# ArchDD/CPP-Raytracer-Rasterizer

Hardware: AMD Instinct MI355X
Metric: Mrays/s (primary+shadow) (higher is better)
Workload: dtype f32

## Files before the change

### cpp-raytracer-rasterizer_amd/capi/binned.cpp

```cpp
#include "capi.hpp"

namespace mirt {


int ensure_pairs(RtScratch &S, size_t cap)
{
    int r;
    if ((r = dev_realloc(&S.d_entries, cap)) || (r = dev_realloc(&S.d_pair_keys, cap)) || (r = dev_realloc(&S.d_pair_vals, cap)) ||
        (r = dev_realloc(&S.d_sorted_keys, cap)) || (r = dev_realloc(&S.d_tmp_vals, cap))) { S.cap_entries = 0; return r; }
    S.cap_entries = (uint32_t)cap;
    return MIRT_OK;
}

constexpr uint32_t BIN_MAX_KEYS = BUCKET_SORT_MAX_BUCKETS * 1024u - 1u;

void poll_pair_count(RtScratch &S)
{
    if (S.count_pending && hipEventQuery(S.ev_count) == hipSuccess) {
        S.known_pairs = *S.h_count; S.have_known = true; S.count_pending = false;
    }
    (void)hipGetLastError();
}

int bin_pass(RtScratch &S, BinSet bs, const OriginRow *cam_tab, const OriginRow *light_tab, uint32_t *counter, uint32_t *bin_off,
             bool fresh, uint32_t *npairs, bool may_guess = false)
{
    int rc;
    poll_pair_count(S);
    if (!fresh && may_guess && S.have_known && S.known_pairs > S.cap_used) fresh = true;
    const bool guess = fresh && may_guess && S.have_known;
    if (!S.d_entries || !S.cap_entries) {
        static const size_t initial = [] { const long v = env_int("MIRT_BIN_INITIAL_PAIRS", 0); return v > 0 ? (size_t)v : (size_t)1 << 20; }();
        if ((rc = ensure_pairs(S, initial))) return rc;
    }
    if (bs.nbins > BIN_MAX_KEYS) return fail(MIRT_ERR_INVALID_ARGUMENT, "binning: %u sort keys exceed the %u the bucket sort holds", bs.nbins, BIN_MAX_KEYS);
    bs.chunk_tris = 256;
    const dim3 bin_grid((unsigned)std::min<long long>((long long)((g.n + bs.chunk_tris - 1) / bs.chunk_tris) * bs.nframes, (long long)g.cu_count * 8));
    bs.counters = counter;
    const uint32_t nbuckets = bucket_sort_buckets(bs.nbins);
    if (nbuckets + 1 > S.cap_buckets) {
        S.cap_buckets = 0;
        if ((rc = dev_realloc(&S.d_bucket, (size_t)3 * (nbuckets + 1)))) return rc;
        HIP_TRY(hipMemsetAsync(S.d_bucket, 0, sizeof(uint32_t) * 3 * (nbuckets + 1), g.stream));
        S.cap_buckets = nbuckets + 1;
        S.bucket_dirty = false;
    }
    uint32_t *bcnt = S.d_bucket, *bbase = S.d_bucket + S.cap_buckets, *bcur = S.d_bucket + 2 * (size_t)S.cap_buckets;
    bs.bucket_cnt = bcnt; bs.nbuckets = nbuckets; bs.bucket_shift = bucket_sort_shift(bs.nbins);
    const size_t bin_lds = (size_t)nbuckets * sizeof(uint32_t);
    {
        static const bool once = [] {
            (void)hipFuncSetAttribute(reinterpret_cast<const void *>(&k_bin_pairs<512>), hipFuncAttributeMaxDynamicSharedMemorySize, 48 * 1024);
            (void)hipFuncSetAttribute(reinterpret_cast<const void *>(&k_bin_pairs<256>), hipFuncAttributeMaxDynamicSharedMemorySize, 48 * 1024);
            return true; }();
        (void)once;
    }
    static const int bin_wg_env = (int)env_int("MIRT_BIN_WG", 0);
    const int bin_wg = (bin_wg_env == 256 || bin_wg_env == 512) ? bin_wg_env : ((g.n < 400000 && g.in_flight >= 3) ? 256 : 512);
    if (guess) {
        const size_t want = (size_t)S.known_pairs + S.known_pairs / 2 + 4096;
        if (want > S.cap_entries) {
            HIP_TRY(hipStreamSynchronize(g.stream));
            if ((rc = ensure_pairs(S, want + want / 4))) return rc;
        }
    }
    bool publish_count = false;
    for (int attempt = 0; attempt < 2; attempt++) {
        static const uint32_t test_cap = [] { const long v = env_int("MIRT_TEST_PAIR_CAP", 0); return v > 0 ? (uint32_t)v : 0u; }();
        S.cap_used = (guess && test_cap && test_cap < S.cap_entries) ? test_cap : S.cap_entries;
        BinPairs pairs = { S.d_pair_keys, S.d_pair_vals, S.cap_used };
        bs.entries = S.d_entries; bs.cap_entries = S.cap_used;
        if (attempt) HIP_TRY(hipMemsetAsync(counter, 0, 4, g.stream));
        if (attempt || S.bucket_dirty) HIP_TRY(hipMemsetAsync(S.d_bucket, 0, sizeof(uint32_t) * 3 * (size_t)S.cap_buckets, g.stream));
        S.bucket_dirty = true;
        if (bin_wg == 256) hipLaunchKernelGGL(k_bin_pairs<256>, bin_grid, dim3(256), bin_lds, g.stream, g.d_tris, cam_tab, light_tab, g.n, bs, pairs);
        else hipLaunchKernelGGL(k_bin_pairs<512>, bin_grid, dim3(512), bin_lds, g.stream, g.d_tris, cam_tab, light_tab, g.n, bs, pairs);
        if (!fresh) break;
        if (guess) {
            if (!S.h_count) {
                HIP_TRY(hipHostMalloc(reinterpret_cast<void **>(&S.h_count), 64, hipHostMallocDefault));
                HIP_TRY(hipEventCreateWithFlags(&S.ev_count, hipEventDisableTiming));
            }
            if (!S.count_pending) publish_count = true;
            *npairs = S.known_pairs;
            break;
        }
        uint32_t total = 0;
        HIP_TRY(hipStreamSynchronize(g.stream));
        HIP_TRY(hipMemcpy(&total, counter, 4, hipMemcpyDeviceToHost));
        *npairs = total;
        S.known_pairs = total; S.have_known = true;
// ... 285 lines not shown
        bs.frame0.nshell = okr ? ns : 1;
        bs.frame0.shell_d0 = (float)dn;
        bs.frame0.shell_iw = okr ? (float)(ns / (df - dn)) : 0.0f;
    }
    const uint32_t cam_keys = (uint32_t)bs.frame0.nbu * (uint32_t)band_tile_rows * (uint32_t)bs.frame0.nshell;
    const int tshells = transient ? light_shells_for(nlights, cube_bins, 0u) : 1;
    const uint32_t per_light = 6u * (uint32_t)(cube_bins * cube_bins) * (uint32_t)tshells;
    bs.nbins = cam_keys;
    if (bs.nbins + 1 > S.cap_bins) {
        const size_t cap = (size_t)bs.nbins + 1;
        HIP_TRY(hipStreamSynchronize(g.stream));
        if ((rc = dev_realloc(&S.d_bin_off, cap))) { S.cap_bins = 0; return rc; }
        S.cap_bins = (uint32_t)cap;
        S.bin_key_valid = false;
    }
    if (!S.d_bin_counters) { HIP_TRY(hipMalloc(reinterpret_cast<void **>(&S.d_bin_counters), 512)); HIP_TRY(hipMemsetAsync(S.d_bin_counters, 0, 512, g.stream)); }
    if (S.sel_n != g.n) {
        HIP_TRY(hipStreamSynchronize(g.stream));
        S.sel_n = 0;
        if ((rc = dev_realloc(&S.d_sel, (size_t)g.n))) return rc;
        S.sel_n = g.n;
        S.bin_key_valid = false;
    }
    bs.bin_off = S.d_bin_off;

    uint64_t key = 0xcbf29ce484222325ull ^ g.scene_version;
    {
        auto mix = [&](const void *p, size_t nb) { const unsigned char *b = (const unsigned char *)p; for (size_t i = 0; i < nb; i++) { key ^= b[i]; key *= 0x100000001b3ull; } };
        mix(view, sizeof *view); mix(&y0, 4); mix(&y1, 4); mix(&g.n, 4); mix(&g.aa, 4);
    }
    const int bin_mode = 0;
// ... 18 lines not shown
        forked = !reuse && !side_off;
        if (forked) {
            HIP_TRY(hipEventRecord(ss.ev_fork, main_stream));
            HIP_TRY(hipStreamWaitEvent(ss.aux, ss.ev_fork, 0));
            g.stream = ss.aux;
        }
        rc = transient_light_pass(L, f, origins, nlights, cube_bins, tshells, per_light, lkey, &lights_kept, reuse ? g.d_hits : nullptr);
        g.stream = main_stream;
        if (rc) return rc;
        if (forked) HIP_TRY(hipEventRecord(ss.ev_join, ss.aux));
    }
    if (reuse) {
        if (!(transient && !lights_kept)) HIP_TRY(hipMemsetAsync(g.d_hits, 0, HIT_BYTES, g.stream));
        g.stats.bins_reused = 1;
    } else {
        S.sel_parity ^= 1;
        SelectOut so;
        memset(&so, 0, sizeof so);
        so.cam_tab = S.d_cam_tab; so.sel = S.d_sel;
        so.sel_count = S.d_bin_counters + SEL_COUNT0 + S.sel_parity; so.sel_count_next = S.d_bin_counters + SEL_COUNT0 + (S.sel_parity ^ 1);
        so.zero_hits = g.d_hits; so.zero_counter = S.d_bin_counters;
        if ((rc = hist_prepare(S, bs.frame0, &so))) return rc;
        const unsigned sel_grid = (unsigned)std::min<long long>(((long long)g.n + 1023) / 1024, (long long)g.cu_count);
        hipLaunchKernelGGL(k_prep_select, dim3(sel_grid), dim3(1024), 0, g.stream, g.d_tris, g.n, bs.frame0, so);
        if ((rc = hist_publish(S))) return rc;
        bs.sel = S.d_sel; bs.sel_count = so.sel_count;
        g.stats_sel_count = so.sel_count;
        if ((rc = bin_pass(S, bs, S.d_cam_tab, nullptr, S.d_bin_counters, S.d_bin_off, true, &S.bin_entries, may_guess))) return rc;
        S.last_bin_mode = bin_mode;
        S.bin_key = key;
        S.bin_key_valid = true;
        if ((size_t)order_seg > S.cap_order) {
            HIP_TRY(hipStreamSynchronize(g.stream));
            S.cap_order = 0;
            if ((rc = dev_realloc(&S.d_order, (size_t)ORDER_GROUPS * ORDER_CLASSES * order_seg))) return rc;
            S.cap_order = order_seg;
        }
        hipLaunchKernelGGL(k_tile_order, dim3((pairs_x + 63) / 64, (unsigned)(bs.frame0.j1 - bs.frame0.j0)), dim3(64), 0, g.stream, cam_off, bs.frame0.nshell,
                           bs.frame0.nbu, bs.frame0.j0, bs.frame0.j1, S.d_bin_counters, S.cap_used, S.d_order, order_seg);
    }
    if (forked) HIP_TRY(hipStreamWaitEvent(g.stream, ss.ev_join, 0));
    k_end(MIRT_K_BIN);

    bp->cam_off = cam_off;
    bp->tiles_x = bs.frame0.nbu;
    bp->cam_shells = bs.frame0.nshell;
    bp->order_seg = order_seg;
    bp->transient = transient;
    bp->cube_bins = cube_bins;
    bp->light_shells = transient ? tshells : g.lc.shells;
    return MIRT_OK;
}

int hist_only_pass(const mirt_view *view)
{
    int rc;
    g.stream = g.cur().stream;
    RtScratch &S = g.cur().rt;
    if (S.cam_tab_n != g.n) {
        S.cam_tab_n = 0;
        if ((rc = dev_realloc(&S.d_cam_tab, (size_t)g.n))) return rc;
        S.cam_tab_n = g.n;
    }
    if (S.sel_n != g.n) {
        HIP_TRY(hipStreamSynchronize(g.stream));
        S.sel_n = 0;
        if ((rc = dev_realloc(&S.d_sel, (size_t)g.n))) return rc;
        S.sel_n = g.n;
    }
    if (!S.d_bin_counters) { HIP_TRY(hipMalloc(reinterpret_cast<void **>(&S.d_bin_counters), 512)); HIP_TRY(hipMemsetAsync(S.d_bin_counters, 0, 512, g.stream)); }
    S.bin_key_valid = false;
    const BinFrameDesc fr = make_camera_frame(view, 0, 0, g.aa);
    SelectOut so;
    memset(&so, 0, sizeof so);
    so.cam_tab = S.d_cam_tab; so.sel = S.d_sel;
    so.sel_count = S.d_bin_counters + HIST_SEL_COUNT; so.sel_count_next = S.d_bin_counters + HIST_SEL_COUNT + 1;
    if ((rc = hist_prepare(S, fr, &so))) return rc;
    if (!g.hist_armed) return MIRT_OK;
    HIP_TRY(hipMemsetAsync(so.sel_count, 0, 4, g.stream));
    const unsigned sel_grid = (unsigned)std::min<long long>(((long long)g.n + 1023) / 1024, (long long)g.cu_count);
    if (sel_grid) hipLaunchKernelGGL(k_prep_select, dim3(sel_grid), dim3(1024), 0, g.stream, g.d_tris, g.n, fr, so);
    HIP_TRY(hipGetLastError());
    return hist_publish(S);
}

int binned_trace(const RtFrame &f, RtScratch &S, RtScratch &L, const BinnedPass &bp)
{
    const bool transient = bp.transient;
    RtTraceFrame tf;
    memset(&tf, 0, sizeof tf);
    tf.f = f;
    tf.f.cam_tab = S.d_cam_tab;
    tf.f.light_tab = transient ? L.d_light_tab : g.lc.d_light_tab;
    tf.f.unsafe = nullptr;
    tf.cam_off = bp.cam_off;
    tf.cam_entries = S.d_entries;
    tf.sel = S.d_sel; tf.sel_count = S.d_bin_counters + SEL_COUNT0 + S.sel_parity;
    static const int lazy_env = (int)env_int("MIRT_LAZY_GEO", -1);
    tf.lazy_geo = lazy_env >= 0 ? (lazy_env != 0) : (g.n >= 400000);
    tf.geo = g.d_geo;
    tf.shade = g.d_shade;
    tf.light_off = transient ? L.d_bin_off : g.lc.d_off;
    tf.light_rows = transient ? L.d_light_rows : g.lc.d_rows;
    tf.light_tri = transient ? L.d_entries : g.lc.d_row_tri;
    tf.light_frames = transient ? L.d_frames : g.lc.d_frames;
    tf.tiles_x = bp.tiles_x;
    tf.cube_bins = bp.cube_bins;
    tf.cam_shells = bp.cam_shells;
    tf.light_shells = bp.light_shells;
    tf.pair_count = S.d_bin_counters;
    tf.pair_cap = S.cap_used;
    tf.light_pair_count = transient ? L.d_bin_counters : nullptr;
    tf.light_pair_cap = L.cap_used;
    tf.order = S.d_order; tf.order_count = S.d_bin_counters + 16; tf.order_seg = bp.order_seg;
    const dim3 tgrid(ORDER_GROUPS * bp.order_seg);
    const size_t lds = rt_trace_lds_bytes(1);
    k_begin(MIRT_K_TRACE);
    g.pending_counted = g.profiling;
    if (f.aa > 1) {
        if (g.profiling) hipLaunchKernelGGL((k_rt_trace2<true, true>), tgrid, dim3(64), lds, g.stream, tf);
        else hipLaunchKernelGGL((k_rt_trace2<true, false>), tgrid, dim3(64), lds, g.stream, tf);
    } else {
        static const int waves5_env = (int)env_int("MIRT_TR_WAVES5", -1);
        const bool waves5 = waves5_env >= 0 ? (waves5_env != 0) : (g.n >= 400000 || g.in_flight <= 2);
        if (g.profiling) hipLaunchKernelGGL((k_rt_trace2<false, true>), tgrid, dim3(64), lds, g.stream, tf);
        else if (waves5) hipLaunchKernelGGL((k_rt_trace2<false, false, 5>), tgrid, dim3(64), lds, g.stream, tf);
        else hipLaunchKernelGGL((k_rt_trace2<false, false>), tgrid, dim3(64), lds, g.stream, tf);
    }
    k_end(MIRT_K_TRACE);
// ... 12 lines not shown
```

### cpp-raytracer-rasterizer_amd/capi/capi.hpp

```cpp
#pragma once

#include "../csrc/bin_sort.hpp"
#include "../csrc/comm.hpp"
#include "../csrc/cull.hpp"
#include "../csrc/dof.hpp"
#include "../csrc/rt_common.hpp"
#include "../csrc/raster_common.hpp"
#include "../csrc/rt_binned.hpp"
#include "../csrc/scan.hpp"
#include "env.hpp"

#include <cstdarg>
#include <cstdio>
#include <cstdlib>
#include <cstring>
#include <algorithm>
#include <cmath>
#include <vector>

#define MIRT_KERNEL __attribute__((global))

namespace mirt {

MIRT_KERNEL void k_prep_origin(const float *, int, const float *, v3, int, OriginRow *, OriginRow *, uint32_t *, unsigned long long *, uint32_t *);
template <int P> MIRT_KERNEL void k_rt_brute(const RtFrame);
template <int P> MIRT_KERNEL void k_rt_small(const RtFrame, int);
MIRT_KERNEL void k_rt_wave(const RtFrame);
struct RtTileFrame {
    RtFrame f;
    BinFrameDesc cam;
    int tiles_x, tiles_y;
    unsigned long long *clear_hits;
    float4 *tables;
};
MIRT_KERNEL void k_tile_tables(const RtTileFrame);
template <int TW, bool AA> MIRT_KERNEL void k_rt_tile2(const RtTileFrame);
template <int WG> MIRT_KERNEL void k_bin_pairs(const float *, const OriginRow *, const OriginRow *, int, BinSet, BinPairs);
struct TilePairRec { uint32_t tile, beg, nA, nB; };
constexpr int ORDER_CLASSES = 8, ORDER_GROUPS = 8;
struct RtTraceFrame {
    RtFrame f;
    const uint32_t *cam_off;
    const uint32_t *cam_entries;
    const GeoRow *geo;
    const ShadeRow *shade;
    const uint32_t *light_off;
    const LightRow *light_rows;
    const uint32_t *light_tri;
    const BinFrameDesc *light_frames;
    int tiles_x;
    int cube_bins;
    int cam_shells;
// ... 19 lines not shown
size_t rt_trace_lds_bytes(int waves);
int launch_raster(RasterFrame &f, RasterScratch &s, uint64_t scene_version, hipStream_t stream, hipEvent_t *ev, bool *ev_used);

extern char g_err[512];
int fail(int code, const char *fmt, ...);

#define HIP_TRY(expr)                                                                          \
    do {                                                                                       \
        hipError_t e_ = (expr);                                                                \
        if (e_ != hipSuccess)                                                                  \
            return fail(MIRT_ERR_HIP, "%s failed: %s (%s:%d)", #expr, hipGetErrorString(e_), __FILE__, __LINE__); \
    } while (0)

enum { EV_CALL0 = 0, EV_CALL1 = 1, EV_K0 = 2, EV_COUNT = 2 + 2 * 8 };
constexpr int MAX_FLIGHT = 4;
constexpr int SEL_COUNT0 = 80;
constexpr int HIST_SEL_COUNT = 82;
constexpr int HIST_RING = 4;
constexpr int HIST_SLOTS = HIST_RING + 1;
constexpr size_t HIT_BYTES = sizeof(unsigned long long) * HIT_SHARDS * HIT_SHARD_STRIDE;

struct RtScratch {
    OriginRow *d_cam_tab = nullptr;
    OriginRow *d_light_tab = nullptr;
    int cam_tab_n = 0, light_tab_n = 0, light_tab_lights = 0;
    float *d_origins = nullptr;
    uint32_t *d_flags = nullptr;
    BinFrameDesc *d_frames = nullptr;
    uint32_t *d_bin_off = nullptr, *d_bin_counters = nullptr;
    uint32_t *d_entries = nullptr;
    uint32_t *d_pair_keys = nullptr, *d_pair_vals = nullptr, *d_sorted_keys = nullptr;
    uint32_t *d_tmp_vals = nullptr;
// ... 6 lines not shown
    bool count_event_due = false;
    bool have_known = false;
    uint32_t known_pairs = 0;
    uint32_t cap_bins = 0, cap_entries = 0;
    uint32_t cap_used = 0;
    uint64_t bin_key = 0;
    uint32_t bin_entries = 0;
    bool bin_key_valid = false;
    LightRow *d_light_rows = nullptr;
    uint32_t cap_light_rows = 0;
    TilePairRec *d_order = nullptr;
    uint32_t cap_order = 0;
    int last_bin_mode = -1;
    uint32_t *d_sel = nullptr;
    int sel_n = 0;
    int sel_parity = 0;
    uint32_t *d_face_sel = nullptr;
    size_t cap_face_sel = 0;
    uint32_t *d_face_counts = nullptr;
    uint32_t *d_hist = nullptr;
    uint32_t *h_hist = nullptr;
    hipEvent_t ev_hist[HIST_SLOTS] = {};
    uint64_t hist_key[HIST_SLOTS] = {};
    uint64_t hist_seq[HIST_SLOTS] = {};
    int hist_rows[HIST_SLOTS] = {}, hist_shift[HIST_SLOTS] = {};
    int hist_next = 0;

    void forget_scene() { bin_key_valid = false; have_known = false; count_pending = false; }
    void release();
};

// ... 146 lines not shown
    int tiles_x, cam_shells;
    uint32_t order_seg;
    bool transient;
    int cube_bins, light_shells;
};
int binned_pass(const RtFrame &f, const mirt_view *view, RtScratch &S, RtScratch &L, const float *origins, int nlights, int y0, int y1, BinnedPass *bp);
int binned_trace(const RtFrame &f, RtScratch &S, RtScratch &L, const BinnedPass &bp);
bool rt_bins_whole_frame(const mirt_view *view, const mirt_light *lights, int nlights, int mode);
int hist_only_pass(const mirt_view *view);

int raster_enqueue(const mirt_view *view, const mirt_light *lights, int nlights, const float *indirect,
                   int y0, int y1, int row_origin, void *d_xrgb, int pitch_bytes, void *d_rgb, void *d_zinv,
                   void *d_index, void *d_fd = nullptr);
int cull_copy_wait_readers(int dst, hipStream_t st);

int hist_prepare(RtScratch &S, const BinFrameDesc &cam, SelectOut *so);
int hist_publish(RtScratch &S);
const uint32_t *hist_lookup(uint64_t max_key, int *rows, int *shift);
void current_bounds(int world, int W, int H, std::vector<int> &bounds);
unsigned part_tile_weight();
int plan_out(int world, int root, int width, int height, int nviews, int strip_rows, const int *bounds, uint64_t *root_offset,
             uint64_t *band_offset, uint64_t *bytes, int32_t *peer, int max_pieces);
int render_sharded(const mirt_view *views, int nviews, int root, void *d_frames, int pitch_bytes, bool raster,
                   const mirt_light *lights, int nlights, const float *indirect, int mode);

struct HostPlane { void *host; void **staging; size_t bpp; };
int ensure_staging(size_t px, const HostPlane *planes, int nplanes);
char *registered_alias(const void *host, size_t pitch, int H);
bool host_direct();
int copy_plane_interior(void *dst, int dst_pitch, const void *src, int src_pitch, int W, int H);
// ... 66 lines not shown
```

### cpp-raytracer-rasterizer_amd/capi/sharded.cpp

```cpp
#include "capi.hpp"

namespace mirt {

static bool hist_wanted() { return g.in_sharded ? g.hist_call : (g.want_hist || g.strip_rows == MIRT_PARTITION_WEIGHTED); }
static int hist_shift_for(int tile_rows) { int sh = 0; while (((tile_rows - 1) >> sh) + 1 > SEL_HIST_MAX) sh++; return sh; }
static int hist_slot(const RtScratch &S) { return g.in_sharded ? S.hist_next : HIST_RING; }
int hist_prepare(RtScratch &S, const BinFrameDesc &cam, SelectOut *so)
{
    g.hist_armed = false;
    if (!hist_wanted()) return MIRT_OK;
    if (!S.d_hist) {
        HIP_TRY(hipMalloc(reinterpret_cast<void **>(&S.d_hist), sizeof(uint32_t) * SEL_HIST_MAX));
        HIP_TRY(hipMemsetAsync(S.d_hist, 0, sizeof(uint32_t) * SEL_HIST_MAX, g.stream));
        HIP_TRY(hipHostMalloc(reinterpret_cast<void **>(&S.h_hist), sizeof(uint32_t) * SEL_HIST_MAX * HIST_SLOTS, hipHostMallocDefault));
        for (int i = 0; i < HIST_SLOTS; i++) HIP_TRY(hipEventCreateWithFlags(&S.ev_hist[i], hipEventDisableTiming));
    }
    so->hist = S.d_hist;
    so->hist_shift = hist_shift_for(cam.nbv);
    const int slot = hist_slot(S);
    S.hist_key[slot] = 0;
    S.hist_rows[slot] = ((cam.nbv - 1) >> so->hist_shift) + 1;
    S.hist_shift[slot] = so->hist_shift;
    g.hist_armed = true;
    return MIRT_OK;
// ... 160 lines not shown
```

### cpp-raytracer-rasterizer_amd/csrc/bin_bucket_sort.hip

```cpp
#include "bin_sort.hpp"

#include <algorithm>
#include <cstdlib>

namespace mirt {

constexpr int BS_PER_THREAD = 16;
constexpr int BS_CHUNK = 256 * BS_PER_THREAD;
constexpr int BS_LOCAL_PER_THREAD = 16;
constexpr int BS_MAX_SHIFT = 12;
constexpr int BS_MAX_BUCKET_KEYS = 1 << BS_MAX_SHIFT;

__device__ __forceinline__ uint32_t bs_block_scan(uint32_t v, uint32_t *s_wave , uint32_t *total)
{
    const int lane = threadIdx.x & 63, wave = threadIdx.x >> 6;
    uint32_t incl = v;
#pragma unroll
    for (int d = 1; d < 64; d <<= 1) {
        const uint32_t o = __shfl_up(incl, d);
        if (lane >= d) incl += o;
    }
    __syncthreads();
    if (lane == 63) s_wave[wave] = incl;
    __syncthreads();
// ... 64 lines not shown
__global__ __launch_bounds__(256) void k_bs_local(const uint32_t *__restrict__ keys, const uint32_t *__restrict__ vals,
                                                  const uint32_t *__restrict__ total_ptr, uint32_t cap,
                                                  const uint32_t *__restrict__ bucket_base, uint32_t nbins, int shift,
                                                  uint32_t *__restrict__ bucket_cnt, uint32_t *__restrict__ cursor,
                                                  uint32_t *__restrict__ bin_off, uint32_t *__restrict__ entries)
{
    __shared__ uint32_t s_cnt[BS_MAX_BUCKET_KEYS], s_wave[4];
    const uint32_t bucket = blockIdx.x;
    if (threadIdx.x == 0) { bucket_cnt[bucket] = 0u; cursor[bucket] = 0u; }
    if (*total_ptr > cap) return;
    const uint32_t beg = bucket_base[bucket], end = bucket_base[bucket + 1];
    const uint32_t nb = 1u << shift, mask = nb - 1u;
    for (uint32_t i = threadIdx.x; i < nb; i += 256) s_cnt[i] = 0u;
    __syncthreads();
    const bool small = end - beg <= 256u * BS_LOCAL_PER_THREAD;
    uint32_t lo[BS_LOCAL_PER_THREAD], v[BS_LOCAL_PER_THREAD], rank[BS_LOCAL_PER_THREAD];
    if (small) {
#pragma unroll
        for (int j = 0; j < BS_LOCAL_PER_THREAD; j++) {
            const uint32_t i = beg + threadIdx.x + 256u * j;
            lo[j] = 0xFFFFFFFFu; v[j] = 0u; rank[j] = 0u;
            if (i < end) { lo[j] = keys[i] & mask; v[j] = vals[i]; }
        }
#pragma unroll
        for (int j = 0; j < BS_LOCAL_PER_THREAD; j++)
            if (lo[j] != 0xFFFFFFFFu) rank[j] = atomicAdd(&s_cnt[lo[j]], 1u);
    } else {
        for (uint32_t i = beg + threadIdx.x; i < end; i += 256) atomicAdd(&s_cnt[keys[i] & mask], 1u);
    }
    __syncthreads();
    uint32_t carry = beg;
    for (uint32_t i0 = 0; i0 < nb; i0 += 256) {
        const uint32_t i = i0 + threadIdx.x;
        const uint32_t c = i < nb ? s_cnt[i] : 0u;
        uint32_t all;
        const uint32_t excl = carry + bs_block_scan(c, s_wave, &all);
        if (i < nb) {
            s_cnt[i] = excl;
            const uint32_t bin = (bucket << shift) + i;
            if (bin <= nbins) bin_off[bin] = excl;
        }
        carry += all;
    }
    __syncthreads();
    if (small) {
#pragma unroll
        for (int j = 0; j < BS_LOCAL_PER_THREAD; j++)
            if (lo[j] != 0xFFFFFFFFu) entries[s_cnt[lo[j]] + rank[j]] = v[j];
    } else {
        for (uint32_t i = beg + threadIdx.x; i < end; i += 256) {
            const uint32_t at = atomicAdd(&s_cnt[keys[i] & mask], 1u);
            entries[at] = vals[i];
        }
    }
}

int bucket_sort_shift(uint32_t nbins)
{
    int shift = 8;
    while (shift < BS_MAX_SHIFT && ((nbins + 1u + (1u << shift) - 1u) >> shift) > 1024u) shift++;
    while (shift > 4 && ((nbins + 1u + (1u << shift) - 1u) >> shift) < 512u) shift--;
    return shift;
}
// ... 21 lines not shown
```

### cpp-raytracer-rasterizer_amd/csrc/rt_binned.hip

```cpp
#include "rt_binned.hpp"

#include <float.h>

namespace mirt {

constexpr int BIN_L0 = BIN_COARSE * BIN_COARSE;

struct BinItem {
    float A0[4], A1[4], A2[4], Bu[4], Bv[4];
    float lou, hiu, lov, hiv;
};

__device__ __forceinline__ float bcastf(float v, int lane) { return __builtin_bit_cast(float, __builtin_amdgcn_readlane(__builtin_bit_cast(int, v), lane)); }

__device__ __forceinline__ float corner(float s, float lo, float hi) { return fmaxf(s * lo, s * hi); }

__device__ __forceinline__ bool cell_may_hit(const BinItem &u, const float (&A)[4], float I, float J, float K)
{
    bool ok = true;
#pragma unroll
    for (int k = 0; k < 4; k++) ok = ok && (__builtin_fmaf(J, u.Bv[k], __builtin_fmaf(I, u.Bu[k], A[k])) >= 0.0f);
    return ok && (I + K >= u.lou) && (I <= u.hiu) && (J + K >= u.lov) && (J <= u.hiv);
}

// ... 231 lines not shown
        for (int f = 0; f < 6; f++) {
            const unsigned long long m = __builtin_amdgcn_ballot_w64((keep >> f) & 1u);
            if (m) {
                uint32_t at0 = 0;
                if (lane == 0) at0 = atomicAdd(&s_fill[f], (uint32_t)__popcll(m));
                at0 = (uint32_t)__builtin_amdgcn_readfirstlane((int)at0);
                if ((keep >> f) & 1u) s_sel[f][at0 + (uint32_t)__popcll(m & ((1ull << lane) - 1ull))] = (uint32_t)i;
            }
        }
        __syncthreads();
    }
    flush();
}


template <int WG>
__global__ __launch_bounds__(WG) void k_bin_pairs(const float *__restrict__ tris15, const OriginRow *__restrict__ cam_tab,
                                                   const OriginRow *__restrict__ light_tab, int n, BinSet bs, BinPairs out)
{
    extern __shared__ uint32_t s_bucket[];
    __shared__ uint32_t s_keys[BIN_PAIR_BUF], s_vals[BIN_PAIR_BUF];
    __shared__ float4 s_A2[256], s_Bu[256], s_Bv[256], s_box[256];
    __shared__ uint32_t s_org[256];
    __shared__ uint32_t s_ni[256];
    __shared__ uint32_t s_tri[256];
    __shared__ uint32_t s_pre[257];
    __shared__ uint32_t s_wave[4];
    __shared__ uint32_t s_base, s_fill, s_valid;
    const int lane = threadIdx.x & 63, wave = threadIdx.x >> 6;
    const int chunk_tris = bs.chunk_tris;
    const int nchunks = (n + chunk_tris - 1) / chunk_tris;
    const bool listed = bs.sel != nullptr;
    const uint32_t nsel = listed ? min(*bs.sel_count, (uint32_t)n) : 0u;
    const int cam_chunk = (listed && nsel < 32768u) ? 64 : chunk_tris;
    const int ncam = listed ? (int)((nsel + (uint32_t)cam_chunk - 1u) / (uint32_t)cam_chunk) : 0;
    const int nrest = listed ? bs.nframes - 1 : bs.nframes;
    const bool faces_listed = bs.face_lists != nullptr;
    __shared__ uint32_t s_first[MAX_BIN_FRAMES + 1];
    if (faces_listed) {
        if (threadIdx.x == 0) {
            uint32_t run = 0;
            for (int ff = 0; ff < nrest; ff++) { s_first[ff] = run; run += (min(bs.face_counts[ff], (uint32_t)n) + (uint32_t)chunk_tris - 1u) / (uint32_t)chunk_tris; }
            s_first[nrest] = run;
        }
        __syncthreads();
    }
    const int nwork = ncam + (faces_listed ? (int)s_first[nrest] : nchunks * nrest);
    if (threadIdx.x == 0) { s_fill = 0u; s_valid = (uint32_t)BIN_PAIR_BUF; }
    if (bs.bucket_cnt)
        for (uint32_t b = threadIdx.x; b < bs.nbuckets; b += WG) s_bucket[b] = 0u;

    auto flush = [&]() {
// ... 50 lines not shown
        BinFrameGrid gr;
        gr.nbu = fr.nbu; gr.fj0 = fr.j0; gr.fj1 = fr.j1; gr.fbase = fr.base; gr.nshell = (uint32_t)max(fr.nshell, 1);
        gr.cells_x = (gr.nbu + BIN_L0 - 1) / BIN_L0; gr.cy0 = gr.fj0 / BIN_L0;
        gr.ncell = gr.cells_x * ((gr.fj1 + BIN_L0 - 1) / BIN_L0 - gr.cy0);
        const int nbu = gr.nbu, fj0 = gr.fj0, fj1 = gr.fj1;
        BinItem it;
        memset(&it, 0, sizeof it);
        int kind = 0;
#ifdef MIRT_BIN_STATS
        int dbg_state = 0;
#endif
        int i_lo = 0, i_hi = -1, j_lo = 0, j_hi = -1;
        unsigned long long cells = 0;
        uint32_t shell = 0;
        if (tri < (uint32_t)n && fj1 > fj0) {
            const OriginRow &row = (fr.tab == 0) ? cam_tab[tri] : light_tab[(size_t)(fr.tab - 1) * n + tri];
            shell = bin_shell_of(fr, row.r1.w);
            TriBinFns t = make_bin_fns(row, fr);
            add_bbox(t, tris15 + (size_t)15 * tri, fr);
#ifdef MIRT_BIN_STATS
            dbg_state = t.bstate == BOX_VALID ? 0 : (t.bstate == BOX_NONE ? 1 : 2);
#endif
            const float T = 1.6940658945086007e-21f;
            const bool both = fabsf(t.nb) < T || !(t.nb == t.nb);
            const float sgn = t.nb < 0.0f ? -1.0f : 1.0f;
            const EdgeFn *fn[4] = { &t.n, &t.p, &t.q, &t.s };
            const float inf = __builtin_huge_valf();
#pragma unroll
            for (int k = 0; k < 4; k++) {
                const float su = sgn * fn[k]->cu, sv = sgn * fn[k]->cv;
                const float base = sgn * fn[k]->c0 + fn[k]->m + su * fr.ulo + sv * fr.vlo;
// ... 24 lines not shown
                    const int cx = c % gr.cells_x, cy = gr.cy0 + c / gr.cells_x;
                    if (cell_may_hit(it, it.A0, (float)(cx * BIN_L0), (float)(cy * BIN_L0), (float)BIN_L0)) cells |= 1ull << c;
                }
                if (gr.ncell > 64) cells = ~0ull;
                if (!cells) kind = 0;
                if (kind == 2 && !both) {
                    BinLin G[4];
#pragma unroll
                    for (int k = 0; k < 4; k++) { G[k].a = sgn * fn[k]->c0 + fn[k]->m; G[k].bu = sgn * fn[k]->cu; G[k].bv = sgn * fn[k]->cv; }
                    const float u0 = fr.ulo + fr.pad_lo, u1 = fr.ulo + (float)nbu * fr.du + fr.pad_hi;
                    const float v0 = fr.vlo + (float)fj0 * fr.dv + fr.pad_lo, v1 = fr.vlo + (float)fj1 * fr.dv + fr.pad_hi;
                    if (bin_jointly_empty(G, u0, u1, v0, v1)) kind = 0;
                }
            }
        }



        STAMP(st_setup)
        const uint32_t ni = (uint32_t)(i_hi - i_lo + 1);
        const uint32_t nb = kind == 1 ? ni * (uint32_t)(j_hi - j_lo + 1) : 0u;
        uint32_t incl = nb;
#pragma unroll
        for (int d = 1; d < 64; d <<= 1) {
            const uint32_t o = __shfl_up(incl, d);
            if (lane >= d) incl += o;
        }
        __syncthreads();
        if (lane == 63 && wave < 4) s_wave[wave] = incl;
        if (kind == 1) {
            s_A2[threadIdx.x] = make_float4(it.A2[0], it.A2[1], it.A2[2], it.A2[3]);
            s_Bu[threadIdx.x] = make_float4(it.Bu[0], it.Bu[1], it.Bu[2], it.Bu[3]);
            s_Bv[threadIdx.x] = make_float4(it.Bv[0], it.Bv[1], it.Bv[2], it.Bv[3]);
            s_box[threadIdx.x] = make_float4(it.lou, it.hiu, it.lov, it.hiv);
            s_org[threadIdx.x] = (uint32_t)i_lo | ((uint32_t)j_lo << 16);
            s_ni[threadIdx.x] = ni | (shell << 8);
            s_tri[threadIdx.x] = tri;
        }
        __syncthreads();
        const uint32_t t0w = s_wave[0], t1w = s_wave[1], t2w = s_wave[2], t3w = s_wave[3];
        if (threadIdx.x < 256) s_pre[threadIdx.x] = (wave > 0 ? t0w : 0u) + (wave > 1 ? t1w : 0u) + (wave > 2 ? t2w : 0u) + incl - nb;
        const uint32_t T = t0w + t1w + t2w + t3w;
        if (threadIdx.x == 0) s_pre[256] = T;

#ifdef MIRT_BIN_STATS
        if (kind == 2) { atomicAdd(&bs.counters[11 + dbg_state], 1u); if (frame == 0) atomicAdd(&bs.counters[14], 1u); }
        if (threadIdx.x == 0) { atomicAdd(&bs.counters[8], T); atomicMax(&bs.counters[9], T); }
        { const unsigned long long md = __ballot(kind == 1); if (lane == 0) atomicAdd(&bs.counters[10], (uint32_t)__popcll(md)); }
#endif
        STAMP(st_prefix)
        constexpr int TPT = BIN_TESTS_PER_THREAD;
        for (uint32_t r0 = 0; r0 < T; r0 += WG * TPT) {
#ifdef MIRT_BIN_STAMPS
            st_nrounds++;
#endif
            __syncthreads();
            if (s_fill + (uint32_t)(WG * TPT) > (uint32_t)BIN_PAIR_BUF) flush();
            bool pass[TPT];
// ... 32 lines not shown
            if (cnt) {
                uint32_t at0 = 0;
                if (lane == 0) at0 = atomicAdd(&s_fill, cnt);
                at0 = (uint32_t)__builtin_amdgcn_readfirstlane((int)at0);
#pragma unroll
                for (int q = 0; q < TPT; q++)
                    if (pass[q]) {
                        const uint32_t at = at0 + off[q] + (uint32_t)__popcll(m[q] & ((1ull << lane) - 1ull));
                        s_keys[at] = key[q]; s_vals[at] = val[q];
                    }
            }
        }

        STAMP(st_rounds)
        __syncthreads();
        {
            BinLargeSink sink = { s_keys, s_vals, &s_fill, &s_valid, &bs.counters[0], out, bs.bucket_cnt, bs.bucket_shift };
            for (unsigned long long ml = __ballot(kind == 2); ml;) {
                const int src = __builtin_ctzll(ml);
                ml &= ml - 1ull;
                BinItem u;
#pragma unroll
                for (int k = 0; k < 4; k++) {
                    u.A0[k] = bcastf(it.A0[k], src); u.A1[k] = bcastf(it.A1[k], src); u.A2[k] = bcastf(it.A2[k], src);
                    u.Bu[k] = bcastf(it.Bu[k], src); u.Bv[k] = bcastf(it.Bv[k], src);
                }
                u.lou = bcastf(it.lou, src); u.hiu = bcastf(it.hiu, src); u.lov = bcastf(it.lov, src); u.hiv = bcastf(it.hiv, src);
                const uint32_t utri = (uint32_t)__builtin_amdgcn_readlane((int)tri, src);
                const uint32_t ushell = (uint32_t)__builtin_amdgcn_readlane((int)shell, src);
                const unsigned long long ucells = ((unsigned long long)(uint32_t)__builtin_amdgcn_readlane((int)(cells >> 32), src) << 32) | (uint32_t)__builtin_amdgcn_readlane((int)cells, src);
// ... 2 lines not shown
        }
        STAMP(st_huge)
    }
#ifdef MIRT_BIN_STAMPS
    st_t = __builtin_amdgcn_s_memtime();
#endif
    flush();
    STAMP(st_flush)
#ifdef MIRT_BIN_STAMPS
    if (threadIdx.x == 0 && (blockIdx.x % 97) == 0)
        printf("wg %d: total %lld | setup %lld prefix %lld rounds %lld (%d) huge %lld flush %lld\n", (int)blockIdx.x, (long long)__builtin_amdgcn_s_memtime() - st_begin,
               st_setup, st_prefix, st_rounds, st_nrounds, st_huge, st_flush);
#endif
}

template __global__ void k_bin_pairs<512>(const float *, const OriginRow *, const OriginRow *, int, BinSet, BinPairs);
template __global__ void k_bin_pairs<256>(const float *, const OriginRow *, const OriginRow *, int, BinSet, BinPairs);

}
```

### cpp-raytracer-rasterizer_amd/csrc/rt_binned.hpp

```cpp
#pragma once

#include "rt_common.hpp"

namespace mirt {

#ifndef MIRT_ORDER_STRIPE_SHIFT
#define MIRT_ORDER_STRIPE_SHIFT 2
#endif
constexpr int ORDER_STRIPE_SHIFT = MIRT_ORDER_STRIPE_SHIFT;
constexpr int BIN_TILE = 8;
constexpr int BIN_COARSE = 8;
constexpr int CUBE_BINS_MIN = 64;
constexpr int MAX_BIN_FRAMES = 1 + 6 * MIRT_MAX_LIGHTS;

struct BinFrameDesc {
    float P0[3], Pu[3], Pv[3];
    float S[3];
    float ru[3], rv[3], rw[3];
    float ulo, vlo, du, dv;
    float pad_lo, pad_hi;
    float dmax;
    int nbu, nbv;
    int j0, j1;
    uint32_t base;
// ... 19 lines not shown
    int nframes;
    uint32_t nbins;
    uint32_t *bin_off;
    uint32_t *entries;
    uint32_t cap_entries;
    uint32_t *counters;
    uint32_t *bucket_cnt;
    uint32_t nbuckets;
    int bucket_shift;
    int chunk_tris;
    const uint32_t *sel;
    const uint32_t *sel_count;
    const uint32_t *face_lists;
    const uint32_t *face_counts;
    uint32_t face_stride;
};

constexpr int SEL_HIST_MAX = 256;
struct SelectOut {
    OriginRow *cam_tab;
    uint32_t *sel;
    uint32_t *sel_count;
    uint32_t *sel_count_next;
    uint32_t *hist;
    int hist_shift;
    uint32_t *zero_faces;
    int zero_faces_n;
    unsigned long long *zero_hits;
    uint32_t *zero_counter;
};

// ... 199 lines not shown
```

Baseline: 47490.

## Fuse camera select pass into bin kernel and double-buffer bin counters

Adds a FUSED variant of the binning kernel that computes each triangle's origin row inline, writes the camera table and the compacted selection list itself, and zeroes the hit buffer and next-frame counters. This lets whole-frame camera binning for scenes under a size threshold skip the separate k_prep_select launch. Counters are moved to a double-buffered block that is reset with an explicit memset when dirty. The fused path also uses smaller triangle chunks for small scenes, and the bucket-sort local path stops early past the occupied slots. The trade-off is extra work and global writes inside the bin kernel and the loss of the selection-list ordering that the later stages previously got.

```diff
diff --git a/cpp-raytracer-rasterizer_amd/capi/binned.cpp b/cpp-raytracer-rasterizer_amd/capi/binned.cpp
--- a/cpp-raytracer-rasterizer_amd/capi/binned.cpp
+++ b/cpp-raytracer-rasterizer_amd/capi/binned.cpp
@@ -35,6 +35,8 @@
     }
     if (bs.nbins > BIN_MAX_KEYS) return fail(MIRT_ERR_INVALID_ARGUMENT, "binning: %u sort keys exceed the %u the bucket sort holds", bs.nbins, BIN_MAX_KEYS);
     bs.chunk_tris = 256;
+    const bool fused = bs.fused_tab != nullptr;
+    if (fused && g.n < 32768) bs.chunk_tris = 64;
     const dim3 bin_grid((unsigned)std::min<long long>((long long)((g.n + bs.chunk_tris - 1) / bs.chunk_tris) * bs.nframes, (long long)g.cu_count * 8));
     bs.counters = counter;
     const uint32_t nbuckets = bucket_sort_buckets(bs.nbins);
@@ -50,8 +52,10 @@
     const size_t bin_lds = (size_t)nbuckets * sizeof(uint32_t);
     {
         static const bool once = [] {
-            (void)hipFuncSetAttribute(reinterpret_cast<const void *>(&k_bin_pairs<512>), hipFuncAttributeMaxDynamicSharedMemorySize, 48 * 1024);
-            (void)hipFuncSetAttribute(reinterpret_cast<const void *>(&k_bin_pairs<256>), hipFuncAttributeMaxDynamicSharedMemorySize, 48 * 1024);
+            (void)hipFuncSetAttribute(reinterpret_cast<const void *>(&k_bin_pairs<512, false>), hipFuncAttributeMaxDynamicSharedMemorySize, 48 * 1024);
+            (void)hipFuncSetAttribute(reinterpret_cast<const void *>(&k_bin_pairs<256, false>), hipFuncAttributeMaxDynamicSharedMemorySize, 48 * 1024);
+            (void)hipFuncSetAttribute(reinterpret_cast<const void *>(&k_bin_pairs<512, true>), hipFuncAttributeMaxDynamicSharedMemorySize, 48 * 1024);
+            (void)hipFuncSetAttribute(reinterpret_cast<const void *>(&k_bin_pairs<256, true>), hipFuncAttributeMaxDynamicSharedMemorySize, 48 * 1024);
             return true; }();
         (void)once;
     }
@@ -70,11 +74,14 @@
         S.cap_used = (guess && test_cap && test_cap < S.cap_entries) ? test_cap : S.cap_entries;
         BinPairs pairs = { S.d_pair_keys, S.d_pair_vals, S.cap_used };
         bs.entries = S.d_entries; bs.cap_entries = S.cap_used;
-        if (attempt) HIP_TRY(hipMemsetAsync(counter, 0, 4, g.stream));
+        if (attempt) HIP_TRY(hipMemsetAsync(counter, 0, fused ? sizeof(uint32_t) * (BIN_CTR_SEL + 1) : 4, g.stream));
         if (attempt || S.bucket_dirty) HIP_TRY(hipMemsetAsync(S.d_bucket, 0, sizeof(uint32_t) * 3 * (size_t)S.cap_buckets, g.stream));
         S.bucket_dirty = true;
-        if (bin_wg == 256) hipLaunchKernelGGL(k_bin_pairs<256>, bin_grid, dim3(256), bin_lds, g.stream, g.d_tris, cam_tab, light_tab, g.n, bs, pairs);
-        else hipLaunchKernelGGL(k_bin_pairs<512>, bin_grid, dim3(512), bin_lds, g.stream, g.d_tris, cam_tab, light_tab, g.n, bs, pairs);
+        if (fused) {
+            if (bin_wg == 256) hipLaunchKernelGGL((k_bin_pairs<256, true>), bin_grid, dim3(256), bin_lds, g.stream, g.d_tris, cam_tab, light_tab, g.n, bs, pairs);
+            else hipLaunchKernelGGL((k_bin_pairs<512, true>), bin_grid, dim3(512), bin_lds, g.stream, g.d_tris, cam_tab, light_tab, g.n, bs, pairs);
+        } else if (bin_wg == 256) hipLaunchKernelGGL((k_bin_pairs<256, false>), bin_grid, dim3(256), bin_lds, g.stream, g.d_tris, cam_tab, light_tab, g.n, bs, pairs);
+        else hipLaunchKernelGGL((k_bin_pairs<512, false>), bin_grid, dim3(512), bin_lds, g.stream, g.d_tris, cam_tab, light_tab, g.n, bs, pairs);
         if (!fresh) break;
         if (guess) {
             if (!S.h_count) {
@@ -390,7 +397,7 @@
         S.cap_bins = (uint32_t)cap;
         S.bin_key_valid = false;
     }
-    if (!S.d_bin_counters) { HIP_TRY(hipMalloc(reinterpret_cast<void **>(&S.d_bin_counters), 512)); HIP_TRY(hipMemsetAsync(S.d_bin_counters, 0, 512, g.stream)); }
+    if (!S.d_bin_counters) { HIP_TRY(hipMalloc(reinterpret_cast<void **>(&S.d_bin_counters), CAM_COUNTER_BYTES)); HIP_TRY(hipMemsetAsync(S.d_bin_counters, 0, CAM_COUNTER_BYTES, g.stream)); }
     if (S.sel_n != g.n) {
         HIP_TRY(hipStreamSynchronize(g.stream));
         S.sel_n = 0;
@@ -439,19 +446,33 @@
         if (!(transient && !lights_kept)) HIP_TRY(hipMemsetAsync(g.d_hits, 0, HIT_BYTES, g.stream));
         g.stats.bins_reused = 1;
     } else {
-        S.sel_parity ^= 1;
-        SelectOut so;
-        memset(&so, 0, sizeof so);
-        so.cam_tab = S.d_cam_tab; so.sel = S.d_sel;
-        so.sel_count = S.d_bin_counters + SEL_COUNT0 + S.sel_parity; so.sel_count_next = S.d_bin_counters + SEL_COUNT0 + (S.sel_parity ^ 1);
-        so.zero_hits = g.d_hits; so.zero_counter = S.d_bin_counters;
-        if ((rc = hist_prepare(S, bs.frame0, &so))) return rc;
-        const unsigned sel_grid = (unsigned)std::min<long long>(((long long)g.n + 1023) / 1024, (long long)g.cu_count);
-        hipLaunchKernelGGL(k_prep_select, dim3(sel_grid), dim3(1024), 0, g.stream, g.d_tris, g.n, bs.frame0, so);
-        if ((rc = hist_publish(S))) return rc;
-        bs.sel = S.d_sel; bs.sel_count = so.sel_count;
-        g.stats_sel_count = so.sel_count;
-        if ((rc = bin_pass(S, bs, S.d_cam_tab, nullptr, S.d_bin_counters, S.d_bin_off, true, &S.bin_entries, may_guess))) return rc;
+        if (S.ctr_dirty) HIP_TRY(hipMemsetAsync(S.d_bin_counters, 0, CAM_COUNTER_BYTES, g.stream));
+        S.ctr_dirty = true;
+        S.bin_key_valid = false;
+        S.ctr_parity ^= 1;
+        uint32_t *ctr = S.cam_counters(), *ctr_next = S.d_bin_counters + (size_t)BIN_CTR_WORDS * (S.ctr_parity ^ 1);
+        static const int fused_env = (int)env_int("MIRT_BIN_FUSED", -1);
+        const bool whole = bs.frame0.j0 == 0 && bs.frame0.j1 == bs.frame0.nbv && g.n < 400000;
+        const bool fused = !hist_wanted() && (fused_env >= 0 ? fused_env != 0 : whole);
+        if (fused) {
+            g.hist_armed = false;
+            bs.fused_tab = S.d_cam_tab; bs.fused_sel = S.d_sel; bs.fused_sel_count = ctr + BIN_CTR_SEL;
+            bs.zero_hits = g.d_hits; bs.zero_next = ctr_next;
+        } else {
+            SelectOut so;
+            memset(&so, 0, sizeof so);
+            so.cam_tab = S.d_cam_tab; so.sel = S.d_sel;
+            so.sel_count = ctr + BIN_CTR_SEL; so.sel_count_next = ctr_next + BIN_CTR_SEL;
+            so.zero_hits = g.d_hits; so.zero_counter = ctr_next;
+            if ((rc = hist_prepare(S, bs.frame0, &so))) return rc;
+            const unsigned sel_grid = (unsigned)std::min<long long>(((long long)g.n + 1023) / 1024, (long long)g.cu_count);
+            hipLaunchKernelGGL(k_prep_select, dim3(sel_grid), dim3(1024), 0, g.stream, g.d_tris, g.n, bs.frame0, so);
+            if ((rc = hist_publish(S))) return rc;
+            bs.sel = S.d_sel; bs.sel_count = so.sel_count;
+        }
+        g.stats_sel_count = ctr + BIN_CTR_SEL;
+        if ((rc = bin_pass(S, bs, S.d_cam_tab, nullptr, ctr, S.d_bin_off, true, &S.bin_entries, may_guess))) return rc;
+        S.ctr_dirty = false;
         S.last_bin_mode = bin_mode;
         S.bin_key = key;
         S.bin_key_valid = true;
@@ -462,7 +483,7 @@
             S.cap_order = order_seg;
         }
         hipLaunchKernelGGL(k_tile_order, dim3((pairs_x + 63) / 64, (unsigned)(bs.frame0.j1 - bs.frame0.j0)), dim3(64), 0, g.stream, cam_off, bs.frame0.nshell,
-                           bs.frame0.nbu, bs.frame0.j0, bs.frame0.j1, S.d_bin_counters, S.cap_used, S.d_order, order_seg);
+                           bs.frame0.nbu, bs.frame0.j0, bs.frame0.j1, ctr, S.cap_used, S.d_order, order_seg);
     }
     if (forked) HIP_TRY(hipStreamWaitEvent(g.stream, ss.ev_join, 0));
     k_end(MIRT_K_BIN);
@@ -493,7 +514,7 @@
         if ((rc = dev_realloc(&S.d_sel, (size_t)g.n))) return rc;
         S.sel_n = g.n;
     }
-    if (!S.d_bin_counters) { HIP_TRY(hipMalloc(reinterpret_cast<void **>(&S.d_bin_counters), 512)); HIP_TRY(hipMemsetAsync(S.d_bin_counters, 0, 512, g.stream)); }
+    if (!S.d_bin_counters) { HIP_TRY(hipMalloc(reinterpret_cast<void **>(&S.d_bin_counters), CAM_COUNTER_BYTES)); HIP_TRY(hipMemsetAsync(S.d_bin_counters, 0, CAM_COUNTER_BYTES, g.stream)); }
     S.bin_key_valid = false;
     const BinFrameDesc fr = make_camera_frame(view, 0, 0, g.aa);
     SelectOut so;
@@ -520,7 +541,8 @@
     tf.f.unsafe = nullptr;
     tf.cam_off = bp.cam_off;
     tf.cam_entries = S.d_entries;
-    tf.sel = S.d_sel; tf.sel_count = S.d_bin_counters + SEL_COUNT0 + S.sel_parity;
+    const uint32_t *ctr = S.cam_counters();
+    tf.sel = S.d_sel; tf.sel_count = ctr + BIN_CTR_SEL;
     static const int lazy_env = (int)env_int("MIRT_LAZY_GEO", -1);
     tf.lazy_geo = lazy_env >= 0 ? (lazy_env != 0) : (g.n >= 400000);
     tf.geo = g.d_geo;
@@ -533,11 +555,11 @@
     tf.cube_bins = bp.cube_bins;
     tf.cam_shells = bp.cam_shells;
     tf.light_shells = bp.light_shells;
-    tf.pair_count = S.d_bin_counters;
+    tf.pair_count = ctr;
     tf.pair_cap = S.cap_used;
     tf.light_pair_count = transient ? L.d_bin_counters : nullptr;
     tf.light_pair_cap = L.cap_used;
-    tf.order = S.d_order; tf.order_count = S.d_bin_counters + 16; tf.order_seg = bp.order_seg;
+    tf.order = S.d_order; tf.order_count = ctr + 16; tf.order_seg = bp.order_seg;
     const dim3 tgrid(ORDER_GROUPS * bp.order_seg);
     const size_t lds = rt_trace_lds_bytes(1);
     k_begin(MIRT_K_TRACE);
diff --git a/cpp-raytracer-rasterizer_amd/capi/capi.hpp b/cpp-raytracer-rasterizer_amd/capi/capi.hpp
--- a/cpp-raytracer-rasterizer_amd/capi/capi.hpp
+++ b/cpp-raytracer-rasterizer_amd/capi/capi.hpp
@@ -35,7 +35,7 @@
 };
 MIRT_KERNEL void k_tile_tables(const RtTileFrame);
 template <int TW, bool AA> MIRT_KERNEL void k_rt_tile2(const RtTileFrame);
-template <int WG> MIRT_KERNEL void k_bin_pairs(const float *, const OriginRow *, const OriginRow *, int, BinSet, BinPairs);
+template <int WG, bool FUSED> MIRT_KERNEL void k_bin_pairs(const float *, const OriginRow *, const OriginRow *, int, BinSet, BinPairs);
 struct TilePairRec { uint32_t tile, beg, nA, nB; };
 constexpr int ORDER_CLASSES = 8, ORDER_GROUPS = 8;
 struct RtTraceFrame {
@@ -85,8 +85,9 @@
 
 enum { EV_CALL0 = 0, EV_CALL1 = 1, EV_K0 = 2, EV_COUNT = 2 + 2 * 8 };
 constexpr int MAX_FLIGHT = 4;
-constexpr int SEL_COUNT0 = 80;
+constexpr size_t CAM_COUNTER_BYTES = sizeof(uint32_t) * 2 * BIN_CTR_WORDS;
 constexpr int HIST_SEL_COUNT = 82;
+static_assert(HIST_SEL_COUNT > BIN_CTR_SEL && HIST_SEL_COUNT + 1 < BIN_CTR_WORDS, "hist_only_pass' counters lie in block 0, beside the words a pass zeroes");
 constexpr int HIST_RING = 4;
 constexpr int HIST_SLOTS = HIST_RING + 1;
 constexpr size_t HIT_BYTES = sizeof(unsigned long long) * HIT_SHARDS * HIT_SHARD_STRIDE;
@@ -123,7 +124,9 @@
     int last_bin_mode = -1;
     uint32_t *d_sel = nullptr;
     int sel_n = 0;
-    int sel_parity = 0;
+    int ctr_parity = 0;
+    bool ctr_dirty = false;
+    uint32_t *cam_counters() const { return d_bin_counters + (size_t)BIN_CTR_WORDS * ctr_parity; }
     uint32_t *d_face_sel = nullptr;
     size_t cap_face_sel = 0;
     uint32_t *d_face_counts = nullptr;
@@ -300,6 +303,7 @@
                    void *d_index, void *d_fd = nullptr);
 int cull_copy_wait_readers(int dst, hipStream_t st);
 
+bool hist_wanted();
 int hist_prepare(RtScratch &S, const BinFrameDesc &cam, SelectOut *so);
 int hist_publish(RtScratch &S);
 const uint32_t *hist_lookup(uint64_t max_key, int *rows, int *shift);
diff --git a/cpp-raytracer-rasterizer_amd/capi/sharded.cpp b/cpp-raytracer-rasterizer_amd/capi/sharded.cpp
--- a/cpp-raytracer-rasterizer_amd/capi/sharded.cpp
+++ b/cpp-raytracer-rasterizer_amd/capi/sharded.cpp
@@ -2,7 +2,7 @@
 
 namespace mirt {
 
-static bool hist_wanted() { return g.in_sharded ? g.hist_call : (g.want_hist || g.strip_rows == MIRT_PARTITION_WEIGHTED); }
+bool hist_wanted() { return g.in_sharded ? g.hist_call : (g.want_hist || g.strip_rows == MIRT_PARTITION_WEIGHTED); }
 static int hist_shift_for(int tile_rows) { int sh = 0; while (((tile_rows - 1) >> sh) + 1 > SEL_HIST_MAX) sh++; return sh; }
 static int hist_slot(const RtScratch &S) { return g.in_sharded ? S.hist_next : HIST_RING; }
 int hist_prepare(RtScratch &S, const BinFrameDesc &cam, SelectOut *so)
diff --git a/cpp-raytracer-rasterizer_amd/csrc/bin_bucket_sort.hip b/cpp-raytracer-rasterizer_amd/csrc/bin_bucket_sort.hip
--- a/cpp-raytracer-rasterizer_amd/csrc/bin_bucket_sort.hip
+++ b/cpp-raytracer-rasterizer_amd/csrc/bin_bucket_sort.hip
@@ -102,17 +102,21 @@
     for (uint32_t i = threadIdx.x; i < nb; i += 256) s_cnt[i] = 0u;
     __syncthreads();
     const bool small = end - beg <= 256u * BS_LOCAL_PER_THREAD;
+    const int nslots = __builtin_amdgcn_readfirstlane((int)((end - beg + 255u) >> 8));
     uint32_t lo[BS_LOCAL_PER_THREAD], v[BS_LOCAL_PER_THREAD], rank[BS_LOCAL_PER_THREAD];
     if (small) {
 #pragma unroll
         for (int j = 0; j < BS_LOCAL_PER_THREAD; j++) {
+            if (j >= nslots) break;
             const uint32_t i = beg + threadIdx.x + 256u * j;
             lo[j] = 0xFFFFFFFFu; v[j] = 0u; rank[j] = 0u;
             if (i < end) { lo[j] = keys[i] & mask; v[j] = vals[i]; }
         }
 #pragma unroll
-        for (int j = 0; j < BS_LOCAL_PER_THREAD; j++)
+        for (int j = 0; j < BS_LOCAL_PER_THREAD; j++) {
+            if (j >= nslots) break;
             if (lo[j] != 0xFFFFFFFFu) rank[j] = atomicAdd(&s_cnt[lo[j]], 1u);
+        }
     } else {
         for (uint32_t i = beg + threadIdx.x; i < end; i += 256) atomicAdd(&s_cnt[keys[i] & mask], 1u);
     }
@@ -133,8 +137,10 @@
     __syncthreads();
     if (small) {
 #pragma unroll
-        for (int j = 0; j < BS_LOCAL_PER_THREAD; j++)
+        for (int j = 0; j < BS_LOCAL_PER_THREAD; j++) {
+            if (j >= nslots) break;
             if (lo[j] != 0xFFFFFFFFu) entries[s_cnt[lo[j]] + rank[j]] = v[j];
+        }
     } else {
         for (uint32_t i = beg + threadIdx.x; i < end; i += 256) {
             const uint32_t at = atomicAdd(&s_cnt[keys[i] & mask], 1u);
diff --git a/cpp-raytracer-rasterizer_amd/csrc/rt_binned.hip b/cpp-raytracer-rasterizer_amd/csrc/rt_binned.hip
--- a/cpp-raytracer-rasterizer_amd/csrc/rt_binned.hip
+++ b/cpp-raytracer-rasterizer_amd/csrc/rt_binned.hip
@@ -269,10 +269,18 @@
 }
 
 
-template <int WG>
+template <int WG, bool FUSED>
 __global__ __launch_bounds__(WG) void k_bin_pairs(const float *__restrict__ tris15, const OriginRow *__restrict__ cam_tab,
                                                    const OriginRow *__restrict__ light_tab, int n, BinSet bs, BinPairs out)
 {
+    if constexpr (FUSED) {
+        if (blockIdx.x == 0) {
+            if (bs.zero_hits)
+                for (int g = threadIdx.x; g < HIT_SHARDS * HIT_SHARD_STRIDE; g += WG) bs.zero_hits[g] = 0ull;
+            if (threadIdx.x == 0 || (threadIdx.x >= 16 && threadIdx.x < 80) || threadIdx.x == BIN_CTR_SEL) bs.zero_next[threadIdx.x] = 0u;
+        }
+    }
+    __shared__ uint32_t s_selw[4], s_selbase;
     extern __shared__ uint32_t s_bucket[];
     __shared__ uint32_t s_keys[BIN_PAIR_BUF], s_vals[BIN_PAIR_BUF];
     __shared__ float4 s_A2[256], s_Bu[256], s_Bv[256], s_box[256];
@@ -285,12 +293,12 @@
     const int lane = threadIdx.x & 63, wave = threadIdx.x >> 6;
     const int chunk_tris = bs.chunk_tris;
     const int nchunks = (n + chunk_tris - 1) / chunk_tris;
-    const bool listed = bs.sel != nullptr;
+    const bool listed = !FUSED && bs.sel != nullptr;
     const uint32_t nsel = listed ? min(*bs.sel_count, (uint32_t)n) : 0u;
     const int cam_chunk = (listed && nsel < 32768u) ? 64 : chunk_tris;
     const int ncam = listed ? (int)((nsel + (uint32_t)cam_chunk - 1u) / (uint32_t)cam_chunk) : 0;
     const int nrest = listed ? bs.nframes - 1 : bs.nframes;
-    const bool faces_listed = bs.face_lists != nullptr;
+    const bool faces_listed = !FUSED && bs.face_lists != nullptr;
     __shared__ uint32_t s_first[MAX_BIN_FRAMES + 1];
     if (faces_listed) {
         if (threadIdx.x == 0) {
@@ -371,7 +379,9 @@
         unsigned long long cells = 0;
         uint32_t shell = 0;
         if (tri < (uint32_t)n && fj1 > fj0) {
-            const OriginRow &row = (fr.tab == 0) ? cam_tab[tri] : light_tab[(size_t)(fr.tab - 1) * n + tri];
+            OriginRow row;
+            if constexpr (FUSED) { row = make_origin_row(tris15 + (size_t)15 * tri, V3(fr.S[0], fr.S[1], fr.S[2])); bs.fused_tab[tri] = row; }
+            else row = (fr.tab == 0) ? cam_tab[tri] : light_tab[(size_t)(fr.tab - 1) * n + tri];
             shell = bin_shell_of(fr, row.r1.w);
             TriBinFns t = make_bin_fns(row, fr);
             add_bbox(t, tris15 + (size_t)15 * tri, fr);
@@ -426,8 +436,8 @@
                 }
             }
         }
-
-
+        unsigned long long mkeep = 0;
+        if constexpr (FUSED) mkeep = __ballot(kind != 0);
 
         STAMP(st_setup)
         const uint32_t ni = (uint32_t)(i_hi - i_lo + 1);
@@ -440,6 +450,8 @@
         }
         __syncthreads();
         if (lane == 63 && wave < 4) s_wave[wave] = incl;
+        if constexpr (FUSED)
+            if (lane == 0 && wave < 4) s_selw[wave] = (uint32_t)__popcll(mkeep);
         if (kind == 1) {
             s_A2[threadIdx.x] = make_float4(it.A2[0], it.A2[1], it.A2[2], it.A2[3]);
             s_Bu[threadIdx.x] = make_float4(it.Bu[0], it.Bu[1], it.Bu[2], it.Bu[3]);
@@ -454,6 +466,12 @@
         if (threadIdx.x < 256) s_pre[threadIdx.x] = (wave > 0 ? t0w : 0u) + (wave > 1 ? t1w : 0u) + (wave > 2 ? t2w : 0u) + incl - nb;
         const uint32_t T = t0w + t1w + t2w + t3w;
         if (threadIdx.x == 0) s_pre[256] = T;
+        if constexpr (FUSED) {
+            if (threadIdx.x == 0) {
+                const uint32_t kept = s_selw[0] + s_selw[1] + s_selw[2] + s_selw[3];
+                if (kept) s_selbase = atomicAdd(bs.fused_sel_count, kept);
+            }
+        }
 
 #ifdef MIRT_BIN_STATS
         if (kind == 2) { atomicAdd(&bs.counters[11 + dbg_state], 1u); if (frame == 0) atomicAdd(&bs.counters[14], 1u); }
@@ -516,6 +534,13 @@
 
         STAMP(st_rounds)
         __syncthreads();
+        if constexpr (FUSED) {
+            if (kind != 0) {
+                const uint32_t before = (wave > 0 ? s_selw[0] : 0u) + (wave > 1 ? s_selw[1] : 0u) + (wave > 2 ? s_selw[2] : 0u);
+                const uint32_t at = s_selbase + before + (uint32_t)__popcll(mkeep & ((1ull << lane) - 1ull));
+                if (at < (uint32_t)n) bs.fused_sel[at] = tri;
+            }
+        }
         {
             BinLargeSink sink = { s_keys, s_vals, &s_fill, &s_valid, &bs.counters[0], out, bs.bucket_cnt, bs.bucket_shift };
             for (unsigned long long ml = __ballot(kind == 2); ml;) {
@@ -548,7 +573,9 @@
 #endif
 }
 
-template __global__ void k_bin_pairs<512>(const float *, const OriginRow *, const OriginRow *, int, BinSet, BinPairs);
-template __global__ void k_bin_pairs<256>(const float *, const OriginRow *, const OriginRow *, int, BinSet, BinPairs);
-
-}
+template __global__ void k_bin_pairs<512, false>(const float *, const OriginRow *, const OriginRow *, int, BinSet, BinPairs);
+template __global__ void k_bin_pairs<256, false>(const float *, const OriginRow *, const OriginRow *, int, BinSet, BinPairs);
+template __global__ void k_bin_pairs<512, true>(const float *, const OriginRow *, const OriginRow *, int, BinSet, BinPairs);
+template __global__ void k_bin_pairs<256, true>(const float *, const OriginRow *, const OriginRow *, int, BinSet, BinPairs);
+
+}
diff --git a/cpp-raytracer-rasterizer_amd/csrc/rt_binned.hpp b/cpp-raytracer-rasterizer_amd/csrc/rt_binned.hpp
--- a/cpp-raytracer-rasterizer_amd/csrc/rt_binned.hpp
+++ b/cpp-raytracer-rasterizer_amd/csrc/rt_binned.hpp
@@ -57,7 +57,15 @@
     const uint32_t *face_lists;
     const uint32_t *face_counts;
     uint32_t face_stride;
-};
+    OriginRow *fused_tab;
+    uint32_t *fused_sel;
+    uint32_t *fused_sel_count;
+    unsigned long long *zero_hits;
+    uint32_t *zero_next;
+};
+
+constexpr int BIN_CTR_WORDS = 128;
+constexpr int BIN_CTR_SEL = 80;
 
 constexpr int SEL_HIST_MAX = 256;
 struct SelectOut {
```

Result: faster. 48130 (median of 6 runs) (+1.4%).
